# Sir-Teo/MuZero-Go

Hardware: AMD Instinct MI355X
Metric: MCTS simulations/sec (whole node) + self-play moves/sec, 9x9 Go, 200 sims/move (higher is better)
Workload: dtype fp32

## Files before the change

muzero-go_amd/csrc/mzgo_board.hpp:

```cpp
#pragma once
#include "mzgo_common.hpp"

namespace mzgo {

struct BoardMeta {
  int turn;
  int passed;
  int done;
  int moves;
};

template <class G>
struct BoardLds {
  int8_t* stone;
  uint8_t* invd;
  int* label;
  int* libs;
  int* gsize;
  int* killed;
  int* misc;
};

template <class G>
struct BoardWG {
  static constexpr int SIZE = G::THREADS;
  __device__ static int id() { return tid_local(); }
  __device__ static void sync() { __syncthreads(); }
  __device__ static bool any(int v) { return __syncthreads_or(v) != 0; }
  __device__ static bool leader() { return tid_local() == 0; }
};
template <class G>
__device__ __forceinline__ bool nbr(int c, int d, int& n) {
  const int r = c / G::N, col = c - r * G::N;
  switch (d) {
    case 0: if (r == 0) return false; n = c - G::N; return true;
    case 1: if (r == G::N - 1) return false; n = c + G::N; return true;
    case 2: if (col == 0) return false; n = c - 1; return true;
    default: if (col == G::N - 1) return false; n = c + 1; return true;
  }
}

template <class G, class T, class ClassFn>
__device__ __forceinline__ void label_components(int* label, ClassFn cls) {
  for (int c = T::id(); c < G::CELLS; c += T::SIZE) label[c] = cls(c) ? c : -1;
  T::sync();
  for (int it = 0; it < G::CELLS + 2; ++it) {
    int changed = 0;
    for (int c = T::id(); c < G::CELLS; c += T::SIZE) {
      const int k = cls(c);
      if (!k) continue;
      int m = label[c];
#pragma unroll
      for (int d = 0; d < 4; ++d) {
        int n;
        if (nbr<G>(c, d, n) && cls(n) == k) { int ln = label[n]; m = ln < m ? ln : m; }
      }
      int j = label[m];
      m = j < m ? j : m;
      if (m < label[c]) { label[c] = m; changed = 1; }
    }
    if (!T::any(changed)) break;
  }
}

template <class G, class T>
__device__ __forceinline__ void count_liberties(BoardLds<G>& b, bool sizes) {
  for (int c = T::id(); c < G::CELLS; c += T::SIZE) { b.libs[c] = 0; if (sizes) b.gsize[c] = 0; }
  T::sync();
  for (int c = T::id(); c < G::CELLS; c += T::SIZE) {
    if (b.stone[c]) {
      if (sizes) atomicAdd(&b.gsize[b.label[c]], 1);
      continue;
    }
    int seen[4];
    int ns = 0;
#pragma unroll
    for (int d = 0; d < 4; ++d) {
      int n;
      if (nbr<G>(c, d, n) && b.stone[n]) {
        int l = b.label[n];
        bool dup = false;
        for (int i = 0; i < ns; ++i) dup |= seen[i] == l;
        if (!dup) { seen[ns++] = l; atomicAdd(&b.libs[l], 1); }
      }
    }
  }
  T::sync();
}

template <class G, class T>
__device__ __forceinline__ void compute_invalid(BoardLds<G>& b, int mover, int ko) {
  for (int c = T::id(); c < G::CELLS; c += T::SIZE) {
    uint8_t inv;
    if (b.stone[c]) {
      inv = 1;
    } else {
      bool boxed = true, maybe_bad = false, surely_ok = false;
#pragma unroll
      for (int d = 0; d < 4; ++d) {
        int n;
        if (!nbr<G>(c, d, n)) continue;
        const int s = b.stone[n];
        if (!s) { boxed = false; continue; }
        const int lib = b.libs[b.label[n]];
        if (s - 1 == mover) { maybe_bad |= lib > 1; surely_ok |= lib == 1; }
        else                { maybe_bad |= lib == 1; surely_ok |= lib > 1; }
      }
      inv = (boxed && maybe_bad && !surely_ok) ? 1 : 0;
    }
    b.invd[c] = inv;
  }
  T::sync();
  if (ko >= 0 && T::leader()) b.invd[ko] = 1;
  T::sync();
}

enum : int { BOARD_OK = 0, BOARD_ERR_DONE = 1, BOARD_ERR_INVALID = 2, BOARD_ERR_RANGE = 3 };

template <class G, class T = BoardWG<G>>
__device__ __forceinline__ int board_step(BoardLds<G>& b, BoardMeta& m, int action) {
  if (m.done) return BOARD_ERR_DONE;
  if (action < 0 || action > G::CELLS) return BOARD_ERR_RANGE;
  const int player = m.turn;
  int ko = -1;
  if (action == G::CELLS) {
    if (m.passed) m.done = 1;
    m.passed = 1;
    label_components<G, T>(b.label, [&](int c) { return (int)b.stone[c]; });
    count_liberties<G, T>(b, false);
  } else {
    if (b.invd[action]) return BOARD_ERR_INVALID;
    m.passed = 0;
    if (T::leader()) {
      b.stone[action] = (int8_t)(player + 1);
      bool boxed = true;
      for (int d = 0; d < 4; ++d) {
        int n;
        if (nbr<G>(action, d, n)) boxed &= b.stone[n] == 2 - player;
      }
      b.misc[1] = boxed;
    }
    T::sync();
    label_components<G, T>(b.label, [&](int c) { return (int)b.stone[c]; });
    count_liberties<G, T>(b, true);
    if (T::leader()) {
      int nk = 0;
      for (int d = 0; d < 4; ++d) {
        int n;
        if (!nbr<G>(action, d, n) || b.stone[n] != 2 - player) continue;
        const int l = b.label[n];
        bool dup = false;
        for (int i = 0; i < nk; ++i) dup |= b.killed[i] == l;
        if (!dup && b.libs[l] == 0) b.killed[nk++] = l;
      }
      b.misc[0] = nk;
      b.misc[2] = (nk == 1 && b.misc[1] && b.gsize[b.killed[0]] == 1) ? b.killed[0] : -1;
    }
    T::sync();
    const int nk = b.misc[0];
    ko = b.misc[2];
    if (nk > 0) {
      for (int c = T::id(); c < G::CELLS; c += T::SIZE) {
        if (b.stone[c] == 2 - player) {
          const int l = b.label[c];
          bool dead = false;
          for (int i = 0; i < nk; ++i) dead |= b.killed[i] == l;
          if (dead) b.stone[c] = 0;
        }
      }
      T::sync();
      count_liberties<G, T>(b, false);
    }
  }
  compute_invalid<G, T>(b, player, ko);
  m.turn = 1 - m.turn;
  m.moves += 1;
  return BOARD_OK;
}

template <class G, class T = BoardWG<G>>
__device__ __forceinline__ double board_winning(BoardLds<G>& b, double komi) {
  label_components<G, T>(b.label, [&](int c) { return b.stone[c] == 0 ? 1 : 0; });
  for (int c = T::id(); c < G::CELLS; c += T::SIZE) { b.libs[c] = 0; b.gsize[c] = 0; }
  T::sync();
  for (int c = T::id(); c < G::CELLS; c += T::SIZE) {
    if (b.stone[c]) continue;
    int f = 0;
#pragma unroll
    for (int d = 0; d < 4; ++d) {
      int n;
      if (nbr<G>(c, d, n) && b.stone[n]) f |= b.stone[n];
    }
    if (f) atomicOr(&b.libs[b.label[c]], f);
    atomicAdd(&b.gsize[b.label[c]], 1);
  }
  T::sync();
  int black = 0, white = 0;
  for (int c = T::id(); c < G::CELLS; c += T::SIZE) {
    if (b.stone[c] == 1) black++;
    else if (b.stone[c] == 2) white++;
    else if (b.label[c] == c) {
      if (b.libs[c] == 1) black += b.gsize[c];
      else if (b.libs[c] == 2) white += b.gsize[c];
    }
  }
  if (T::leader()) { b.misc[3] = 0; b.misc[4] = 0; }
  T::sync();
  atomicAdd(&b.misc[3], black);
  atomicAdd(&b.misc[4], white);
  T::sync();
  const double diff = (double)b.misc[3] - (double)b.misc[4] - komi;
  T::sync();
  return diff > 0 ? 1.0 : (diff < 0 ? -1.0 : 0.0);
}

}
```

muzero-go_amd/csrc/mzgo_kernels.hpp:

```cpp
#pragma once
#include "mzgo_jobs.hpp"
#include "mzgo_replay.hpp"

namespace mzgo {

template <class G>
constexpr bool rep_needs_scratch() {
  if constexpr (G::WINO) return Wino<G>::NSTRIP > 1;
  else return false;
}

struct NoRepJobs {
  __device__ bool operator()(int) const { return false; }
};

template <class G, class PlaneFn, class Jobs = NoRepJobs>
__device__ __forceinline__ void representation(Smem<G>& sm, const NetParams& np, PlaneFn planes, float* lat,
                                      int lat_stride, float* scr, unsigned long long* ts = nullptr,
                                      Jobs jobs = Jobs{}) {
  float* mid = rep_needs_scratch<G>() ? scr : lat;
  for (int i = tid_local(); i < 6 * G::CELLS; i += G::THREADS) {
    const int c = i / G::CELLS, j = i - c * G::CELLS;
    sm.u.in[c * G::CPAD + j] = planes(c, j);
  }
// ... 1162 lines not shown
  if (tid_local() == 0) {
    E.nodes[g] = nodes;
    atomicAdd(&E.counters[3], (unsigned long long)(factored ? convs : nodes - 1));
    atomicAdd(&E.counters[5], (unsigned long long)(factored ? rows : nodes - 1));
    if (nbcomp) atomicAdd(&E.counters[9], (unsigned long long)nbcomp);
    if (nbcache) atomicAdd(&E.counters[10], (unsigned long long)nbcache);
    if (ncut) atomicAdd(&E.counters[11], (unsigned long long)ncut);
    if (narr_lds) atomicAdd(&E.counters[12], (unsigned long long)narr_lds);
    if (narr_l2) atomicAdd(&E.counters[13], (unsigned long long)narr_l2);
  }
  __syncthreads();
}

template <class G, class PlaneFn>
__device__ __forceinline__ void run_search(Smem<G>& sm, const NetParams& np, const SearchParams& sp,
                                  const EngineArrays& E, int g, PlaneFn planes, const double* noise,
                                  uint64_t key, unsigned long long* ts = nullptr, double* noise_out = nullptr) {
  const TreeView TV = TreeViewOf<G>::make(E, g);
  if (tid_local() == 0) sm.t.ngrab = 0;
  build_mask<G>(sm.t, sp.pass_epsilon, [&](int a) { return planes(3, a); });
  float* pool = pool_of<G>(E, g);
  const size_t node_floats = (size_t)G::C * G::CS;
  if (sp.factored && shared_jobs<G>(sp))
    representation<G>(sm, np, planes, pool + (size_t)(E.S + 1) * node_floats, G::CS, pool, ts ? ts + 3 : nullptr,
                      [&](int k) { rep_shared<G>(sm, np, E, g, sp.net, k); return true; });
  else if (sp.factored)
    representation<G>(sm, np, planes, pool + (size_t)(E.S + 1) * node_floats, G::CS, pool, ts ? ts + 3 : nullptr);
  else
    representation<G>(sm, np, planes, pool, G::CS, pool + node_floats, ts ? ts + 3 : nullptr);
#ifdef MZGO_STAMPS
  if (ts) ts[0] = __builtin_amdgcn_s_memtime();
#endif
  if (noise) {
    if (wave_id() == 0) root_priors<G>(sm.t, TV, sp, noise, key, nullptr, noise_out);
  } else {
    static_assert(G::AP < G::WAVES, "a wave per 64 Gamma draws besides wave 0");
    draw_dirichlet<G>(sm.t, key, sp.dirichlet_alpha, &sm.t.ngrab);
    if (wave_id() == 0) root_priors<G>(sm.t, TV, sp, noise, key, &sm.t.ngrab, noise_out);
  }
  __syncthreads();
#ifdef MZGO_STAMPS
  if (ts) ts[1] = __builtin_amdgcn_s_memtime();
#endif
  if constexpr (G::TREE_CAP > 0) {
    if (sp.num_simulations + 2 <= G::TREE_CAP) {
      sim_loop<G, TreeAcc<G, true>>(sm, np, sp, E, g, TV, key);
      return;
    }
  }
  sim_loop<G, TreeAcc<G, false>>(sm, np, sp, E, g, TV, key);
}

template <class G>
__device__ __forceinline__ void search_outputs(const EngineArrays& E, int g, int* out_visits, double* out_value) {
  const TreeView T = TreeViewOf<G>::make(E, g);
  for (int a = tid_local(); a < G::A; a += G::THREADS) {
    const int c = T.child[a];
    if (out_visits) out_visits[(size_t)g * G::A + a] = c >= 0 ? T.visits[c] : 0;
  }
  if (tid_local() == 0 && out_value) out_value[g] = root_value(T);
}

template <class G>
__device__ __forceinline__ void settle_all_priors(Smem<G>& sm, const NetParams& np, const EngineArrays& E, int g,
                                                  int nodes, int variant) {
  if constexpr (decltype(sm.u.f)::BATCH && G::TREE_CAP > 0) {
    const TreeView TV = TreeViewOf<G>::make(E, g);
    const float* pool = pool_of<G>(E, g);
    const int wave = __builtin_amdgcn_readfirstlane(wave_id());
    const int lane = lane_id_local();
    auto& W = sm.u.f.wv[wave];
    static_assert(sizeof(W.xw) >= sizeof(float) * G::CELLS, "a wave's head rows hold one node's policy sums");
    const int lim = nodes < G::TREE_CAP ? nodes : G::TREE_CAP;
    if (wave == 0 && lane == 0) sm.t.lognode = -1;
    for (int p = wave; p < lim; p += G::WAVES) {
      if (sm.t.is_raw(p)) continue;
      for (int a0 = 0; a0 < G::A; a0 += 64) {
        const int a = a0 + lane;
        const int c = a < G::A ? TV.child[(size_t)p * G::A + a] : -1;
        for (uint64_t m = __ballot(c > 0 && c < lim && sm.t.is_raw(c)); m; m &= m - 1) {
          const int l = __builtin_ctzll(m);
          const int cc = __builtin_amdgcn_readlane(c, l), ca = a0 + l;
          policy_sums_wave<G>(W.xw, pool + (size_t)p * G::C * G::CS, np.etab + (size_t)ca * 9 * G::C, np.head_w);
          wave_lds_sync();
          float x[G::AP], q[G::AP];
          policy_logits<G>(W.xw, sm.t.hsc, x);
          child_prior_regs<G>(sm.t, x, q, variant, W.fb, W.db);
#pragma unroll
          for (int j = 0; j < G::AP; ++j)
            if (lane + 64 * j < G::A) {
              TV.prior[(size_t)cc * G::A + lane + 64 * j] = q[j];
              TV.child[(size_t)cc * G::A + lane + 64 * j] = -1;
            }
          wave_lds_sync();
        }
      }
    }
    __syncthreads();
    for (int i = tid_local(); i < (G::TREE_CAP + 31) / 32; i += G::THREADS) sm.t.rawp[i] = 0u;
  }
  __syncthreads();
}

template <int N, int C>
__global__ void __launch_bounds__((Geo<N, C>::THREADS)) __attribute__((amdgpu_waves_per_eu(Geo<N, C>::WPE, Geo<N, C>::WPE))) k_search(NetParams np_arg, SearchParams sp, EngineArrays E_arg,
                                                      const float* __restrict__ root_obs,
                                                      const double* __restrict__ noise, int game_base,
                                                      int move_index, int* out_visits, double* out_value) {
  typedef Geo<N, C> G;
  __shared__ Smem<G> sm;
  static_assert(sizeof(Smem<G>) <= 160 * 1024, "one workgroup per CU: the whole LDS at most");
  if constexpr (G::WINO) wino_raw_zero<G>(sm.raw);
  const EngineArrays E = launder_arrays(E_arg);
  const NetParams np = launder_params(np_arg);
  const int g = blockIdx.x;
  const float* o = root_obs + (size_t)g * 6 * G::CELLS;
  const uint64_t key = stream_key(sp.seed, (uint32_t)(game_base + g), (uint32_t)move_index);
  run_search<G>(sm, np, sp, E, g, [&](int c, int j) { return o[c * G::CELLS + j]; },
                noise ? noise + (size_t)g * G::A : nullptr, key);
  settle_all_priors<G>(sm, np, E, g, E.nodes[g], sp.variant);
  search_outputs<G>(E, g, out_visits, out_value);
}

template <class G>
__device__ __forceinline__ void board_reset_slot(const EngineArrays& E, int g) {
  for (int c = tid_local(); c < G::CELLS; c += G::THREADS) {
    E.stones[(size_t)g * G::CELLS + c] = 0;
    E.invd[(size_t)g * G::CELLS + c] = 0;
  }
  if (tid_local() < 4) E.meta[g * 4 + tid_local()] = 0;
  if (tid_local() == 0) { E.status[g] = 0; E.game_len[g] = 0; E.final_reward[g] = 0.0; }
}

template <int N, int C>
__global__ void __launch_bounds__((Geo<N, C>::THREADS)) __attribute__((amdgpu_waves_per_eu(Geo<N, C>::WPE, Geo<N, C>::WPE))) k_board_reset(EngineArrays E) {
  board_reset_slot<Geo<N, C>>(E, blockIdx.x);
}

template <int N, int C>
__global__ void __launch_bounds__((Geo<N, C>::THREADS)) __attribute__((amdgpu_waves_per_eu(Geo<N, C>::WPE, Geo<N, C>::WPE))) k_board_step(EngineArrays E, const int* __restrict__ actions,
                                                          int* status, double* winner, double komi) {
  typedef Geo<N, C> G;
  __shared__ Smem<G> sm;
  static_assert(sizeof(Smem<G>) <= 160 * 1024, "one workgroup per CU: the whole LDS at most");
  const int g = blockIdx.x;
  const int a = actions[g];
  if (a < 0) return;
  BoardMeta m;
  board_load<G>(sm.stone, sm.invd, E, g, m);
  BoardLds<G> b = board_lds<G>(sm);
  const int st = board_step<G>(b, m, a);
  __syncthreads();
  if (st == BOARD_OK) board_store<G>(sm.stone, sm.invd, E, g, m);
  double w = 0.0;
  if (st == BOARD_OK && m.done) w = board_winning<G>(b, komi);
  if (tid_local() == 0) {
    if (status) status[g] = st;
    if (winner) winner[g] = w;
  }
}

template <int N, int C>
__global__ void __launch_bounds__((Geo<N, C>::THREADS)) __attribute__((amdgpu_waves_per_eu(Geo<N, C>::WPE, Geo<N, C>::WPE))) k_board_planes(EngineArrays E, double* planes) {
  typedef Geo<N, C> G;
  const int g = blockIdx.x;
  const int* mm = E.meta + g * 4;
  double* p = planes + (size_t)g * 6 * G::CELLS;
  for (int j = tid_local(); j < G::CELLS; j += G::THREADS) {
    const int s = E.stones[(size_t)g * G::CELLS + j];
    p[j] = s == 1; p[G::CELLS + j] = s == 2; p[2 * G::CELLS + j] = mm[0];
    p[3 * G::CELLS + j] = E.invd[(size_t)g * G::CELLS + j];
    p[4 * G::CELLS + j] = mm[1]; p[5 * G::CELLS + j] = mm[2];
  }
}

template <class G, bool CAPS, class KeyId>
__device__ __forceinline__ bool selfplay_one_move(Smem<G>& sm, const NetParams& np_a_arg, const NetParams& np_b_arg,
                                                  const SearchParams& sp, const PlayParams& pp,
                                                  const EngineArrays& E_arg, int g, KeyId key_id, BoardMeta& m) {
#ifdef MZGO_STAMPS
  unsigned long long tm[8] = {0, 0, 0, 0, 0, 0, 0, 0};
  tm[0] = __builtin_amdgcn_s_memtime();
#else
  unsigned long long* tm = nullptr;
#endif
  const int mv = m.moves;
  const EngineArrays E = launder_arrays(E_arg);
  const NetParams np_a = launder_params(np_a_arg), np_b = launder_params(np_b_arg);
  const NetParams np = select_params(pp.arena && (((pp.game_base + g) + mv) & 1), np_b, np_a);
  const size_t rec = (size_t)g * E.max_moves + mv;
  const uint64_t key = move_key(sp, key_id(), mv);
  const int budget = move_budget<CAPS>(sp, key);
  record_observation<G>(E, rec, sm.stone, sm.invd, m, CAPS && budget != sp.num_simulations);
  const BoardMeta m0 = m;
  const double* noise = pp.noise ? pp.noise + ((size_t)g * E.max_moves + mv) * G::A : nullptr;
  double* noise_out = pp.noise_out ? pp.noise_out + ((size_t)g * E.max_moves + mv) * G::A : nullptr;
#ifdef MZGO_STAMPS
  tm[1] = __builtin_amdgcn_s_memtime();
#endif
  SearchParams spm = launder_search(sp);
  spm.net = (pp.arena && (((pp.game_base + g) + mv) & 1)) ? 1 : 0;
  if constexpr (CAPS) spm.num_simulations = budget;
  run_search<G>(sm, np, spm, E, g, [&](int c, int j) { return board_plane<G>(sm.stone, sm.invd, m0, c, j); },
                noise, key, tm ? tm + 2 : nullptr, noise_out);
#ifdef MZGO_STAMPS
  tm[4] = __builtin_amdgcn_s_memtime();
#endif

  const TreeView T = TreeViewOf<G>::make(E, g);
  if (wave_id() == 0) {
    const int a = choose_move_action<G>(sm.t, T, sp, pp, mv, key, E.rec_policy + rec * G::A);
    if (lane_id_local() == 0) {
      sm.bc[0] = a;
      E.rec_action[rec] = a;
      E.rec_value[rec] = root_value(T);
    }
  }
  __syncthreads();
  BoardLds<G> b = board_lds<G>(sm);
  double w;
  const int st = play_action<G>(E, g, b, m, sm.bc[0], pp.komi, w);
#ifdef MZGO_STAMPS
  if (tid_local() == 0 && E.stamps) {
    const unsigned long long t5 = __builtin_amdgcn_s_memtime();
    unsigned long long* sl = E.stamps + (size_t)blockIdx.x * kStampPhases;
    sl[83] += tm[1] - tm[0];
    sl[84] += tm[2] - tm[1];
    sl[85] += tm[3] - tm[2];
    sl[86] += tm[4] - tm[3];
    sl[87] += t5 - tm[4];
    sl[88] += tm[5] - tm[1];
    sl[89] += tm[6] - tm[5];
    sl[90] += tm[2] - tm[6];
  }
#endif
  return finish_move<G>(E, budget, g, rec, st, m, w);
}

template <int N, int C, bool CAPS = false>
__global__ void __launch_bounds__((Geo<N, C>::THREADS)) __attribute__((amdgpu_waves_per_eu(Geo<N, C>::WPE, Geo<N, C>::WPE))) k_selfplay_move(NetParams np_a_arg, NetParams np_b_arg,
                                                             SearchParams sp, PlayParams pp, EngineArrays E_arg) {
  typedef Geo<N, C> G;
  __shared__ Smem<G> sm;
  static_assert(sizeof(Smem<G>) <= 160 * 1024, "one workgroup per CU: the whole LDS at most");
  const int games = gridDim.x - sp.helpers;
  if ((int)blockIdx.x >= games) {
    if constexpr (Smem<G>::GLOBAL_Y && G::WINO) {
      wino_raw_zero<G>(sm.raw);
      int t = (blockIdx.x - games) % games;
      for (;;) {
        helper_loop<G>(sm, np_a_arg, np_b_arg, sp, E_arg, t);
        if (!sp.tail) break;
        t = join_running_game<G>(sm, E_arg, games, t);
        if (t < 0) break;
      }
    }
    return;
  }
  const int g = blockIdx.x;
  const EngineArrays& E = E_arg;
  if (tid_local() == 0) atomicAdd(&E_arg.counters[6], 1ull);
  auto release_helpers = [&]() {
    if ((sp.helpers > 0 || sp.tail) && tid_local() == 0) job_exit(job_of<G>(E_arg, g));
  };
  auto tail_phase = [&]() {
    if constexpr (Smem<G>::GLOBAL_Y && G::WINO) {
      if (sp.tail) {
        __syncthreads();
        for (int t = g; (t = join_running_game<G>(sm, E_arg, games, t)) >= 0;)
          helper_loop<G>(sm, np_a_arg, np_b_arg, sp, E_arg, t);
      }
    }
    if constexpr (TailConvs<G>::value)
      if (sp.tail) {
        __syncthreads();
#ifdef MZGO_STAMPS
        const unsigned long long th = __builtin_amdgcn_s_memtime();
#endif
        tail_help<G>(sm, np_a_arg, np_b_arg, E_arg, g, games);
#ifdef MZGO_STAMPS
        if (tid_local() == 0 && E_arg.stamps) E_arg.stamps[(size_t)blockIdx.x * kStampPhases + 47] +=
            __builtin_amdgcn_s_memtime() - th;
#endif
      }
  };
  if (E.status[g] != 0) { release_helpers(); tail_phase(); return; }
  if ((sp.helpers > 0 || sp.tail) && tid_local() == 0) job_mark_started(job_of<G>(E_arg, g));
  if constexpr (G::WINO) wino_raw_zero<G>(sm.raw);
  BoardMeta m;
  board_load<G>(sm.stone, sm.invd, E, g, m);
  for (int step = 0; step < pp.moves; ++step) {
    if (selfplay_one_move<G, CAPS>(sm, np_a_arg, np_b_arg, sp, pp, E_arg, g,
                             [&]() { return game_key_id(pp.game_base, g, pp.epoch); }, m))
      break;
    __syncthreads();
  }
  release_helpers();
  tail_phase();
}

template <class G>
struct BoardsGeo {
  static constexpr int THREADS = (G::CELLS + 63) / 64 * 64 < 512 ? (G::CELLS + 63) / 64 * 64 : 512;
};
template <class G>
struct BoardsTeam {
  static constexpr int SIZE = BoardsGeo<G>::THREADS;
  __device__ static int id() { return tid_local(); }
  __device__ static void sync() { __syncthreads(); }
  __device__ static bool any(int v) { return __syncthreads_or(v) != 0; }
  __device__ static bool leader() { return tid_local() == 0; }
};
template <class G>
struct BoardsSmem {
  TreeLds<G> t;
  int label[G::CELLS], libs[G::CELLS], gsize[G::CELLS];
  int8_t stone[G::CELLS];
  uint8_t invd[G::CELLS];
  int killed[4];
  int misc[8];
  int bc[8];
};

template <int N, int C, bool CAPS = false>
__global__ void __launch_bounds__((BoardsGeo<Geo<N, C>>::THREADS)) k_selfplay_boards(SearchParams sp, PlayParams pp,
                                                                                    EngineArrays E) {
  typedef Geo<N, C> G;
  typedef BoardsTeam<G> T;
  __shared__ BoardsSmem<G> sm;
  const int g = blockIdx.x;
  const int tid = tid_local();
  if (tid == 0) {
    atomicAdd(&E.counters[6], 1ull);
    E.mpq[2 * g + 1] = 0;
  }
  if (E.status[g] != 0) return;
  BoardMeta m;
  board_load<G, T>(sm.stone, sm.invd, E, g, m);
  BoardLds<G> b = make_board_lds<G>(sm.stone, sm.invd, sm.label, sm.libs, sm.gsize, sm.killed, sm.misc);
  const int mv_first = m.moves;
  int played = 0;
  const TreeView TV = TreeViewOf<G>::make(E, g);
  for (int step = 0; step < pp.moves; ++step) {
    const int mv = m.moves;
    const size_t rec = (size_t)g * E.max_moves + mv;
    const uint64_t key = move_key(sp, pp, g, mv);
    const int budget = move_budget<CAPS>(sp, key);
    record_observation<G, T>(E, rec, sm.stone, sm.invd, m, CAPS && budget != sp.num_simulations);
    ++played;
    build_mask<G, T>(sm.t, sp.pass_epsilon, [&](int a) { return sm.invd[a]; });
    if (wave_id() == 0) {
      const int a = choose_action<G>(sm.t, TV, sp.compat, move_temperature(pp, mv), key, E.rec_policy + rec * G::A);
      if (lane_id_local() == 0) {
        sm.bc[0] = a;
        E.rec_action[rec] = a;
      }
    }
    __syncthreads();
    double w;
    const int st = play_action<G, T>(E, g, b, m, sm.bc[0], pp.komi, w);
    if (finish_move<G, T>(E, budget, g, rec, st, m, w)) break;
    __syncthreads();
  }
  if (tid == 0) {
    E.mpq[2 * g] = mv_first;
    E.mpq[2 * g + 1] = played;
  }
}

template <int N, int C, bool CAPS = false>
__global__ void __launch_bounds__((Geo<N, C>::THREADS)) __attribute__((amdgpu_waves_per_eu(Geo<N, C>::WPE, Geo<N, C>::WPE))) k_search_queue(NetParams np_arg, SearchParams sp, PlayParams pp,
                                                            EngineArrays E_arg, int games) {
  typedef Geo<N, C> G;
  __shared__ Smem<G> sm;
  static_assert(sizeof(Smem<G>) <= 160 * 1024, "one workgroup per CU: the whole LDS at most");
  if constexpr (G::WINO) wino_raw_zero<G>(sm.raw);
  const int leaders = (int)gridDim.x - sp.helpers;
  if ((int)blockIdx.x >= leaders) {
    if constexpr (Smem<G>::GLOBAL_Y && G::WINO)
      helper_loop<G>(sm, np_arg, np_arg, sp, E_arg, ((int)blockIdx.x - leaders) % leaders);
    return;
  }
  const int slot = blockIdx.x;
  const int items = games * pp.moves;
  for (;;) {
    if (tid_local() == 0) sm.bc[0] = (int)atomicAdd((unsigned*)&E_arg.mpq[2 * games], 1u);
    __syncthreads();
    const int k = sm.bc[0];
    __syncthreads();
    if (k >= items) break;
    const int j = k / games, g = k % games;
    const int mv0 = __builtin_amdgcn_readfirstlane(E_arg.mpq[2 * g]);
    const int nmv = __builtin_amdgcn_readfirstlane(E_arg.mpq[2 * g + 1]);
    if (j >= nmv) continue;
    const int mv = mv0 + nmv - 1 - j;
    const EngineArrays E = launder_arrays(E_arg);
    const NetParams np = launder_params(np_arg);
    const size_t rec = (size_t)g * E.max_moves + mv;
    for (int c = tid_local(); c < G::CELLS; c += G::THREADS) {
      sm.stone[c] = E.rec_stones[rec * G::CELLS + c];
      sm.invd[c] = E.rec_invd[rec * G::CELLS + c];
    }
    const BoardMeta m0 = flags_unpack(E.rec_flags[rec], mv);
    __syncthreads();
    const uint64_t key = move_key(sp, pp, g, mv);
    const double* noise = pp.noise ? pp.noise + rec * G::A : nullptr;
    double* noise_out = pp.noise_out ? pp.noise_out + rec * G::A : nullptr;
    SearchParams spm = launder_search(sp);
    spm.net = 0;
    if constexpr (CAPS) spm.num_simulations = move_budget<CAPS>(sp, key);
    run_search<G>(sm, np, spm, E, slot, [&](int c, int jj) { return board_plane<G>(sm.stone, sm.invd, m0, c, jj); },
                  noise, key, nullptr, noise_out);
    if (tid_local() == 0) E.rec_value[rec] = root_value(TreeViewOf<G>::make(E, slot));
    __syncthreads();
  }
  if (sp.helpers > 0 && tid_local() == 0) job_exit(job_of<G>(E_arg, slot));
}

struct ReanalyseArgs {
  const int8_t* stones;
  const uint8_t* invd;
  const uint8_t* flags;
  const int* ids;
  const double* noise;
  int n;
  unsigned* head;
  int* visits;
  double* value;
  double* policy;
};

template <int N, int C, bool INPLACE = false>
__global__ void __launch_bounds__((Geo<N, C>::THREADS)) __attribute__((amdgpu_waves_per_eu(Geo<N, C>::WPE, Geo<N, C>::WPE))) k_reanalyse_queue(NetParams np_arg, SearchParams sp,
                                                               EngineArrays E_arg, typename std::conditional<INPLACE, ReanalyseStoreArgs, ReanalyseArgs>::type ra) {
  typedef Geo<N, C> G;
  __shared__ Smem<G> sm;
  static_assert(sizeof(Smem<G>) <= 160 * 1024, "one workgroup per CU: the whole LDS at most");
  if constexpr (G::WINO) wino_raw_zero<G>(sm.raw);
  const int slot = blockIdx.x;
  if constexpr (INPLACE) {
    for (;;) {
      if (tid_local() == 0) sm.bc[0] = (int)atomicAdd(ra.head, 1u);
      __syncthreads();
      const int i = sm.bc[0];
      __syncthreads();
      if (i >= *launder_global(ra.n)) break;
      const EngineArrays E = launder_arrays(E_arg);
      const NetParams np = launder_params(np_arg);
      const int* it = launder_global(ra.items) + 2 * (size_t)i;
      const int rs = it[0], t = it[1];
      const size_t q = (size_t)rs * (ra.R.M + 1) + t;
      const int8_t* st = launder_global(ra.R.stones) + q * G::CELLS;
      const uint8_t* iv = launder_global(ra.R.invd) + q * G::CELLS;
      for (int c = tid_local(); c < G::CELLS; c += G::THREADS) {
        sm.stone[c] = st[c];
        sm.invd[c] = iv[c];
      }
      const BoardMeta m0 = flags_unpack(launder_global(ra.R.flags)[q], t);
      __syncthreads();
      const uint64_t key = stream_key(sp.seed, (uint32_t)launder_global(ra.R.key_gid)[rs], (uint32_t)t);
      SearchParams spm = launder_search(sp);
      spm.net = 0;
      spm.helpers = 0;
      run_search<G>(sm, np, spm, E, slot, [&](int c, int jj) { return board_plane<G>(sm.stone, sm.invd, m0, c, jj); },
                    nullptr, key);
      const TreeView T = TreeViewOf<G>::make(E, slot);
      const size_t o = (size_t)rs * ra.R.M + t;
      if (tid_local() == 0) {
        launder_global(ra.R.root_value)[o] = root_value(T);
        uint8_t* fl = launder_global(ra.R.flags) + q;
        if (*fl & kFlagFast) *fl = (uint8_t)(*fl & ~kFlagFast);
      }
      if (wave_id() == 0) {
        double vc[G::AP], msum;
        visit_policy<G>(sm.t, T, sp.variant, 1, launder_global(ra.R.policy) + o * G::A, vc, msum);
      }
      __syncthreads();
    }
  } else
  for (;;) {
    if (tid_local() == 0) sm.bc[0] = (int)atomicAdd(ra.head, 1u);
    __syncthreads();
    const int i = sm.bc[0];
    __syncthreads();
    if (i >= ra.n) break;
    const EngineArrays E = launder_arrays(E_arg);
    const NetParams np = launder_params(np_arg);
    const int8_t* st = launder_global(ra.stones) + (size_t)i * G::CELLS;
    const uint8_t* iv = launder_global(ra.invd) + (size_t)i * G::CELLS;
    for (int c = tid_local(); c < G::CELLS; c += G::THREADS) {
      sm.stone[c] = st[c];
      sm.invd[c] = iv[c];
    }
    const int* id = launder_global(ra.ids) + 2 * (size_t)i;
    const BoardMeta m0 = flags_unpack(launder_global(ra.flags)[i], id[1]);
    __syncthreads();
    const uint64_t key = stream_key(sp.seed, (uint32_t)id[0], (uint32_t)id[1]);
    const double* noise = ra.noise ? launder_global(ra.noise) + (size_t)i * G::A : nullptr;
    SearchParams spm = launder_search(sp);
    spm.net = 0;
    spm.helpers = 0;
    run_search<G>(sm, np, spm, E, slot, [&](int c, int jj) { return board_plane<G>(sm.stone, sm.invd, m0, c, jj); },
                  noise, key);
    const TreeView T = TreeViewOf<G>::make(E, slot);
    int* ov = launder_global(ra.visits) + (size_t)i * G::A;
    for (int a = tid_local(); a < G::A; a += G::THREADS) {
      const int c = T.child[a];
      ov[a] = c >= 0 ? T.visits[c] : 0;
    }
    if (tid_local() == 0) launder_global(ra.value)[i] = root_value(T);
    if (ra.policy && wave_id() == 0) {
      double vc[G::AP], msum;
      visit_policy<G>(sm.t, T, sp.variant, 1, launder_global(ra.policy) + (size_t)i * G::A, vc, msum);
    }
    __syncthreads();
  }
}

template <int N, int C, bool CAPS = false>
__global__ void __launch_bounds__((Geo<N, C>::THREADS)) __attribute__((amdgpu_waves_per_eu(Geo<N, C>::WPE, Geo<N, C>::WPE))) k_selfplay_games(NetParams np_arg, SearchParams sp, PlayParams pp,
                                                              EngineArrays E_arg, GamesArgs ga) {
  typedef Geo<N, C> G;
  __shared__ Smem<G> sm;
  static_assert(sizeof(Smem<G>) <= 160 * 1024, "one workgroup per CU: the whole LDS at most");
  if constexpr (G::WINO) wino_raw_zero<G>(sm.raw);
  const int slot = blockIdx.x;
  if (tid_local() == 0) atomicAdd(&E_arg.counters[6], 1ull);
  for (;;) {
    if (tid_local() == 0) sm.bc[0] = (int)atomicAdd(ga.head, 1u);
    __syncthreads();
    const int j = __builtin_amdgcn_readfirstlane(sm.bc[0]);
    __syncthreads();
    if (j >= ga.n) break;
    const uint32_t kid = game_key_id(pp.game_base, j % ga.G, ga.epoch0 + j / ga.G);
    board_reset_slot<G>(E_arg, slot);
    for (int c = tid_local(); c < G::CELLS; c += G::THREADS) {
      sm.stone[c] = 0;
      sm.invd[c] = 0;
    }
    BoardMeta m{0, 0, 0, 0};
    __syncthreads();
    for (int step = 0; step < pp.moves; ++step) {
      if (selfplay_one_move<G, CAPS>(sm, np_arg, np_arg, sp, pp, E_arg, slot, [&]() { return kid; }, m)) break;
      __syncthreads();
    }
    __syncthreads();
    if (tid_local() == 0 && E_arg.status[slot] >= 16) atomicMin(ga.error, j);
    const ReplayEngineView V{N, ga.G, E_arg.max_moves, C, 0, pp.game_base, 0,
                             E_arg.stones, E_arg.invd, E_arg.meta, E_arg.rec_stones, E_arg.rec_invd,
                             E_arg.rec_flags, E_arg.rec_action, E_arg.rec_value, E_arg.rec_policy,
                             E_arg.rec_reward, E_arg.final_reward};
    replay_ingest_game(ga.R, V, slot, (ga.first + j) % ga.R.cap, (int)kid, tid_local(), G::THREADS);
    __syncthreads();
  }
}

}
```

muzero-go_amd/csrc/mzgo_move.hpp:

```cpp
#pragma once
#include "mzgo_board.hpp"
#include "mzgo_search.hpp"

namespace mzgo {

constexpr int kCounters = 14;

struct EngineArrays {
  int S;
  int max_moves;
  float* pool;
  float* prior;
  int* child;
  int* visits;
  double* wsum;
  double* root_prior;
  int* path;
  int* nodes;
  int* nact;
  double* cval;
  int8_t* stones;
  uint8_t* invd;
  int* meta;
  int8_t* rec_stones;
  uint8_t* rec_invd;
  uint8_t* rec_flags;
  int* rec_action;
  double* rec_value;
  double* rec_policy;
  double* rec_reward;
  int* game_len;
  double* final_reward;
  int* status;
  unsigned char* jobs;
  int* mpq;
  unsigned long long* counters;
  unsigned long long* stamps;
};

struct PlayParams {
  double temperature;
  int temperature_moves;
  double komi;
  int game_base;
  int epoch;
  const double* noise;
  double* noise_out;
  int arena;
  int moves;
};

template <class G>
__device__ __forceinline__ BoardLds<G> make_board_lds(int8_t* stone, uint8_t* invd, int* label, int* libs,
                                                      int* gsize, int* killed, int* misc) {
  return BoardLds<G>{stone, invd, label, libs, gsize, killed, misc};
}

template <class G, class T = BoardWG<G>>
__device__ __forceinline__ void board_load(int8_t* stone, uint8_t* invd, const EngineArrays& E, int g,
                                           BoardMeta& m) {
  for (int c = T::id(); c < G::CELLS; c += T::SIZE) {
    stone[c] = E.stones[(size_t)g * G::CELLS + c];
    invd[c] = E.invd[(size_t)g * G::CELLS + c];
  }
  const int* mm = E.meta + g * 4;
  m.turn = mm[0]; m.passed = mm[1]; m.done = mm[2]; m.moves = mm[3];
  T::sync();
}

template <class G, class T = BoardWG<G>>
__device__ __forceinline__ void board_store(const int8_t* stone, const uint8_t* invd, const EngineArrays& E, int g,
                                            const BoardMeta& m) {
  for (int c = T::id(); c < G::CELLS; c += T::SIZE) {
    E.stones[(size_t)g * G::CELLS + c] = stone[c];
    E.invd[(size_t)g * G::CELLS + c] = invd[c];
  }
  if (T::leader()) {
    int* mm = E.meta + g * 4;
    mm[0] = m.turn; mm[1] = m.passed; mm[2] = m.done; mm[3] = m.moves;
  }
}

template <class G>
__device__ __forceinline__ float board_plane(const int8_t* stone, const uint8_t* invd, const BoardMeta& m, int c,
                                             int j) {
  switch (c) {
    case 0: return stone[j] == 1 ? 1.f : 0.f;
    case 1: return stone[j] == 2 ? 1.f : 0.f;
    case 2: return (float)m.turn;
    case 3: return (float)invd[j];
    case 4: return (float)m.passed;
    default: return (float)m.done;
  }
}

__device__ __forceinline__ uint8_t flags_pack(const BoardMeta& m) {
  return (uint8_t)(m.turn | (m.passed << 1) | (m.done << 2));
}
__device__ __forceinline__ BoardMeta flags_unpack(int fl, int mv) {
  return BoardMeta{fl & 1, (fl >> 1) & 1, (fl >> 2) & 1, mv};
}

constexpr int kFlagFast = 8;

template <class G, class T = BoardWG<G>>
__device__ __forceinline__ void record_observation(const EngineArrays& E, size_t rec, const int8_t* stone,
                                                   const uint8_t* invd, const BoardMeta& m, bool fast = false) {
  for (int c = T::id(); c < G::CELLS; c += T::SIZE) {
    E.rec_stones[rec * G::CELLS + c] = stone[c];
    E.rec_invd[rec * G::CELLS + c] = invd[c];
  }
  if (T::leader()) E.rec_flags[rec] = (uint8_t)(flags_pack(m) | (fast ? kFlagFast : 0));
}

__host__ __device__ __forceinline__ uint32_t game_key_id(int game_base, int g, int epoch) {
  return (uint32_t)(game_base + g) ^ ((uint32_t)epoch << 24);
}
__device__ __forceinline__ uint64_t move_key(const SearchParams& sp, uint32_t kid, int mv) {
  return stream_key(sp.seed, kid, (uint32_t)mv);
}
__device__ __forceinline__ uint64_t move_key(const SearchParams& sp, const PlayParams& pp, int g, int mv) {
  return move_key(sp, game_key_id(pp.game_base, g, pp.epoch), mv);
}

template <bool CAPS>
__device__ __forceinline__ int move_budget(const SearchParams& sp, uint64_t key) {
  if constexpr (!CAPS) return sp.num_simulations;
  else return __builtin_amdgcn_readfirstlane(
      playout_budget(key, sp.num_simulations, sp.fast_simulations, sp.full_search_prob));
}

template <class G, class T = BoardWG<G>, class InvdFn>
__device__ __forceinline__ void build_mask(TreeLds<G>& t, double pass_epsilon, InvdFn invd) {
  int any = 0;
  for (int a = T::id(); a < G::A; a += T::SIZE) {
    uint8_t v = a < G::CELLS ? (invd(a) == 0 ? 1 : 0) : 1;
    t.valid[a] = v;
    any |= (a < G::CELLS) && v;
  }
  any = T::any(any);
  if (T::leader()) t.pass_prior = any ? pass_epsilon : 1.0;
  T::sync();
}

template <class G>
__device__ __forceinline__ int pick_valid(const TreeLds<G>& t, uint64_t h) {
  const int lane = lane_id_local();
  uint64_t vb[G::AP];
  int nvalid = 0;
#pragma unroll
  for (int j = 0; j < G::AP; ++j) {
    const int a = lane + 64 * j;
    vb[j] = __ballot(a < G::A && mask_of<G>(t, a) > 0);
    nvalid += __popcll(vb[j]);
  }
  uint32_t k = randbelow(h, (uint32_t)nvalid);
  int action = -1;
#pragma unroll
  for (int j = 0; j < G::AP; ++j) {
    const uint32_t c = __popcll(vb[j]);
    if (action < 0 && k < c) {
      uint64_t mm = vb[j];
      for (uint32_t i = 0; i < k; ++i) mm &= mm - 1;
      action = 64 * j + __ffsll((long long)mm) - 1;
    } else if (action < 0) {
      k -= c;
    }
  }
  return action;
}

template <class G>
__device__ __forceinline__ int argmax_action(const double (&v)[G::AP]) {
  const int lane = lane_id_local();
  double bv = -1.0;
  int ba = 0x7fffffff, payload = 0;
#pragma unroll
  for (int j = 0; j < G::AP; ++j) {
    const int a = lane + 64 * j;
    if (a < G::A && (v[j] > bv || (v[j] == bv && a < ba))) { bv = v[j]; ba = a; }
  }
  wave_argmax(bv, ba, payload);
  return ba;
}

template <class G>
__device__ __forceinline__ double visit_policy(TreeLds<G>& t, const TreeView& T, int variant, int compat,
                                               double* pol, double (&vc)[G::AP], double& msum) {
  const int lane = lane_id_local();
  if (variant == 1) {
    double tot = 0.0;
#pragma unroll
    for (int j = 0; j < G::AP; ++j) {
      const int a = lane + 64 * j;
      vc[j] = 0.0;
      if (a < G::A && mask_of<G>(t, a) > 0) { const int c = T.child[a]; vc[j] = c >= 0 ? (double)T.visits[c] : 0.0; }
      tot += vc[j];
    }
    tot = wave_sum(tot);
#pragma unroll
    for (int j = 0; j < G::AP; ++j) {
      const int a = lane + 64 * j;
      if (a < G::A) pol[a] = tot > 0 ? vc[j] / tot : 0.0;
    }
    msum = 0.0;
    return tot;
  }
  for (int a = lane; a < G::A; a += 64) {
    double v = 0.0;
    if (compat == 1) { const int c = T.child[a]; v = c >= 0 ? (double)T.visits[c] : 0.0; }
    t.dbuf[a] = v * mask_of<G>(t, a);
  }
  wave_lds_sync();
  const double vsum = np_pairwise_sum<double, G::A>(t.dbuf);
#pragma unroll
  for (int j = 0; j < G::AP; ++j) { const int a = lane + 64 * j; vc[j] = a < G::A ? t.dbuf[a] : 0.0; }
  wave_lds_sync();
  for (int a = lane; a < G::A; a += 64) t.dbuf[a] = mask_of<G>(t, a);
  wave_lds_sync();
  msum = np_pairwise_sum<double, G::A>(t.dbuf);
#pragma unroll
  for (int j = 0; j < G::AP; ++j) {
    const int a = lane + 64 * j;
    if (a < G::A) pol[a] = vsum > 0 ? vc[j] / vsum : mask_of<G>(t, a) / msum;
  }
  return vsum;
}

template <class G>
__device__ __forceinline__ int choose_action_main(TreeLds<G>& t, const TreeView& T, uint64_t key, double* pol) {
  const int lane = lane_id_local();
  double vc[G::AP], msum;
  const double tot = visit_policy<G>(t, T, 1, 1, pol, vc, msum);
  if (tot > 0) return argmax_action<G>(vc);
  const int action = pick_valid<G>(t, draw(key, TAG_ACTION, 0));
#pragma unroll
  for (int j = 0; j < G::AP; ++j) {
    const int a = lane + 64 * j;
    if (a < G::A) pol[a] = a == action ? 1.0 : 0.0;
  }
  return action;
}

template <class G>
__device__ __forceinline__ int choose_action(TreeLds<G>& t, const TreeView& T, int compat, double temperature,
                                    uint64_t key, double* pol) {
  const int lane = lane_id_local();
  double vcm[G::AP], msum;
  const double vsum = visit_policy<G>(t, T, 0, compat, pol, vcm, msum);
  const uint64_t h = draw(key, TAG_ACTION, 0);
  if (temperature == 0.0) return vsum > 0 ? argmax_action<G>(vcm) : pick_valid<G>(t, h);
  const double e = 1.0 / temperature;
#pragma unroll
  for (int j = 0; j < G::AP; ++j) {
    const int a = lane + 64 * j;
    if (a < G::A) t.dbuf[a] = (e == 1.0 ? vcm[j] : pow(vcm[j], e)) * mask_of<G>(t, a);
  }
  wave_lds_sync();
  const double ts = np_pairwise_sum<double, G::A>(t.dbuf);
  wave_lds_sync();
  for (int a = lane; a < G::A; a += 64) t.dbuf[a] = ts > 0 ? t.dbuf[a] / ts : mask_of<G>(t, a) / msum;
  wave_lds_sync();
  if (lane == 0) {
    double cdf = 0.0;
    for (int a = 0; a < G::A; ++a) cdf += t.dbuf[a];
    const double total = cdf;
    const double u = u01(h);
    double run = 0.0;
    int idx = 0;
    for (int a = 0; a < G::A; ++a) {
      run += t.dbuf[a];
      if (run / total <= u) idx = a + 1;
    }
    t.bcast = idx;
  }
  wave_lds_sync();
  return t.bcast;
}

__device__ __forceinline__ double move_temperature(const PlayParams& pp, int mv) {
  return mv < pp.temperature_moves ? pp.temperature : 0.0;
}
template <class G>
__device__ __forceinline__ int choose_move_action(TreeLds<G>& t, const TreeView& T, const SearchParams& sp,
                                                  const PlayParams& pp, int mv, uint64_t key, double* pol) {
  return sp.variant == 1 ? choose_action_main<G>(t, T, key, pol)
                         : choose_action<G>(t, T, sp.compat, move_temperature(pp, mv), key, pol);
}

__device__ __forceinline__ double root_value(const TreeView& T) {
  const int n = T.visits[0];
  return n > 0 ? T.wsum[0] / (double)n : 0.0;
}

template <class G, class T = BoardWG<G>>
__device__ __forceinline__ int play_action(const EngineArrays& E, int g, BoardLds<G>& b, BoardMeta& m, int action,
                                           double komi, double& w) {
  const int st = board_step<G, T>(b, m, action);
  T::sync();
  w = (st == BOARD_OK && m.done) ? board_winning<G, T>(b, komi) : 0.0;
  board_store<G, T>(b.stone, b.invd, E, g, m);
  return st;
}

template <class G, class T = BoardWG<G>>
__device__ __forceinline__ bool finish_move(const EngineArrays& E, int sims, int g, size_t rec, int st,
                                            const BoardMeta& m, double w) {
  const bool ended = m.done || m.moves >= E.max_moves;
  if (T::leader()) {
    E.rec_reward[rec] = w;
    atomicAdd(&E.counters[0], (unsigned long long)sims);
    atomicAdd(&E.counters[1], 1ull);
    if (st != BOARD_OK) {
      E.status[g] = 16 + st;
    } else if (ended) {
      E.status[g] = 1;
      E.game_len[g] = m.moves;
      E.final_reward[g] = m.done ? w : 0.0;
      atomicAdd(&E.counters[2], 1ull);
    }
  }
  return st != BOARD_OK || ended;
}

}
```

Baseline: 143.1 million.

## Incrementally update board groups, lighten barriers, and batch move counters in the board loop

The multi-move board loop now keeps group labels across moves: it merges neighbouring friendly labels directly instead of rerunning iterative connected-component labelling on every stone placement, and the board is stored to global memory only once at the end. The team sync and any-reduction use wave-level syncs or raw s_barrier with per-wave flags instead of __syncthreads/__syncthreads_or. Global atomics for the sim, move and game counters are accumulated locally and flushed once per game. The temperature sampling in choose_action is rewritten as a wave-parallel prefix scan with a ballot instead of a serial lane-0 loop. These changes cut per-move synchronisation, global traffic and labelling passes, at the cost of more complex invariants: labels must stay consistent after captures and passes, and the rewritten CDF summation order may change floating-point rounding.

Result: faster. 144.7 million (median of 6 runs) (+1.2%).

```diff
diff --git a/muzero-go_amd/csrc/mzgo_board.hpp b/muzero-go_amd/csrc/mzgo_board.hpp
--- a/muzero-go_amd/csrc/mzgo_board.hpp
+++ b/muzero-go_amd/csrc/mzgo_board.hpp
@@ -26,7 +26,7 @@
   static constexpr int SIZE = G::THREADS;
   __device__ static int id() { return tid_local(); }
   __device__ static void sync() { __syncthreads(); }
-  __device__ static bool any(int v) { return __syncthreads_or(v) != 0; }
+  __device__ static bool any(int v, int = 0) { return __syncthreads_or(v) != 0; }
   __device__ static bool leader() { return tid_local() == 0; }
 };
 template <class G>
@@ -59,7 +59,7 @@
       m = j < m ? j : m;
       if (m < label[c]) { label[c] = m; changed = 1; }
     }
-    if (!T::any(changed)) break;
+    if (!T::any(changed, it)) break;
   }
 }
 
@@ -117,7 +117,13 @@
 
 enum : int { BOARD_OK = 0, BOARD_ERR_DONE = 1, BOARD_ERR_INVALID = 2, BOARD_ERR_RANGE = 3 };
 
-template <class G, class T = BoardWG<G>>
+template <class G, class T>
+__device__ __forceinline__ void board_groups(BoardLds<G>& b) {
+  label_components<G, T>(b.label, [&](int c) { return (int)b.stone[c]; });
+  count_liberties<G, T>(b, false);
+}
+
+template <class G, class T = BoardWG<G>, bool KEEP = false>
 __device__ __forceinline__ int board_step(BoardLds<G>& b, BoardMeta& m, int action) {
   if (m.done) return BOARD_ERR_DONE;
   if (action < 0 || action > G::CELLS) return BOARD_ERR_RANGE;
@@ -126,11 +132,21 @@
   if (action == G::CELLS) {
     if (m.passed) m.done = 1;
     m.passed = 1;
-    label_components<G, T>(b.label, [&](int c) { return (int)b.stone[c]; });
-    count_liberties<G, T>(b, false);
+    if constexpr (!KEEP) board_groups<G, T>(b);
   } else {
     if (b.invd[action]) return BOARD_ERR_INVALID;
     m.passed = 0;
+    int join[4] = {-2, -2, -2, -2}, lmin = action;
+    if constexpr (KEEP) {
+#pragma unroll
+      for (int d = 0; d < 4; ++d) {
+        int n;
+        if (nbr<G>(action, d, n) && b.stone[n] == player + 1) {
+          join[d] = b.label[n];
+          lmin = join[d] < lmin ? join[d] : lmin;
+        }
+      }
+    }
     if (T::leader()) {
       b.stone[action] = (int8_t)(player + 1);
       bool boxed = true;
@@ -141,7 +157,16 @@
       b.misc[1] = boxed;
     }
     T::sync();
-    label_components<G, T>(b.label, [&](int c) { return (int)b.stone[c]; });
+    if constexpr (KEEP) {
+      for (int c = T::id(); c < G::CELLS; c += T::SIZE) {
+        if (c == action) { b.label[c] = lmin; continue; }
+        if (b.stone[c] != player + 1) continue;
+        const int l = b.label[c];
+        if (l == join[0] || l == join[1] || l == join[2] || l == join[3]) b.label[c] = lmin;
+      }
+    } else {
+      label_components<G, T>(b.label, [&](int c) { return (int)b.stone[c]; });
+    }
     count_liberties<G, T>(b, true);
     if (T::leader()) {
       int nk = 0;
@@ -165,7 +190,7 @@
           const int l = b.label[c];
           bool dead = false;
           for (int i = 0; i < nk; ++i) dead |= b.killed[i] == l;
-          if (dead) b.stone[c] = 0;
+          if (dead) { b.stone[c] = 0; if constexpr (KEEP) b.label[c] = -1; }
         }
       }
       T::sync();
diff --git a/muzero-go_amd/csrc/mzgo_kernels.hpp b/muzero-go_amd/csrc/mzgo_kernels.hpp
--- a/muzero-go_amd/csrc/mzgo_kernels.hpp
+++ b/muzero-go_amd/csrc/mzgo_kernels.hpp
@@ -1488,13 +1488,37 @@
 template <class G>
 struct BoardsGeo {
   static constexpr int THREADS = (G::CELLS + 63) / 64 * 64 < 512 ? (G::CELLS + 63) / 64 * 64 : 512;
+  static constexpr int WAVES = THREADS / 64;
 };
 template <class G>
 struct BoardsTeam {
   static constexpr int SIZE = BoardsGeo<G>::THREADS;
+  static constexpr int WAVES = BoardsGeo<G>::WAVES;
   __device__ static int id() { return tid_local(); }
-  __device__ static void sync() { __syncthreads(); }
-  __device__ static bool any(int v) { return __syncthreads_or(v) != 0; }
+  __device__ static void sync() {
+    if constexpr (WAVES == 1) {
+      wave_lds_sync();
+    } else {
+      __builtin_amdgcn_fence(__ATOMIC_RELEASE, "workgroup", "local");
+      __builtin_amdgcn_s_barrier();
+      __builtin_amdgcn_fence(__ATOMIC_ACQUIRE, "workgroup", "local");
+    }
+  }
+  __device__ static bool any(int v, int phase = 0) {
+    const bool mine = __ballot(v != 0) != 0;
+    if constexpr (WAVES == 1) {
+      wave_lds_sync();
+      return mine;
+    } else {
+      __shared__ int flag[2][WAVES];
+      if (lane_id_local() == 0) flag[phase & 1][wave_id()] = mine;
+      sync();
+      int r = 0;
+#pragma unroll
+      for (int w = 0; w < WAVES; ++w) r |= flag[phase & 1][w];
+      return r != 0;
+    }
+  }
   __device__ static bool leader() { return tid_local() == 0; }
 };
 template <class G>
@@ -1524,8 +1548,20 @@
   BoardMeta m;
   board_load<G, T>(sm.stone, sm.invd, E, g, m);
   BoardLds<G> b = make_board_lds<G>(sm.stone, sm.invd, sm.label, sm.libs, sm.gsize, sm.killed, sm.misc);
+  board_groups<G, T>(b);
+#ifdef MZGO_STAMPS
+  unsigned long long lapc[6] = {}, lapt = __builtin_amdgcn_s_memtime();
+  auto lap = [&](int k) {
+    const unsigned long long now = __builtin_amdgcn_s_memtime();
+    lapc[k] += now - lapt;
+    lapt = now;
+  };
+#else
+  auto lap = [](int) {};
+#endif
   const int mv_first = m.moves;
-  int played = 0;
+  int played = 0, finished = 0;
+  unsigned long long sims = 0;
   const TreeView TV = TreeViewOf<G>::make(E, g);
   for (int step = 0; step < pp.moves; ++step) {
     const int mv = m.moves;
@@ -1533,8 +1569,11 @@
     const uint64_t key = move_key(sp, pp, g, mv);
     const int budget = move_budget<CAPS>(sp, key);
     record_observation<G, T>(E, rec, sm.stone, sm.invd, m, CAPS && budget != sp.num_simulations);
+    lap(0);
     ++played;
+    sims += (unsigned long long)budget;
     build_mask<G, T>(sm.t, sp.pass_epsilon, [&](int a) { return sm.invd[a]; });
+    lap(1);
     if (wave_id() == 0) {
       const int a = choose_action<G>(sm.t, TV, sp.compat, move_temperature(pp, mv), key, E.rec_policy + rec * G::A);
       if (lane_id_local() == 0) {
@@ -1542,13 +1581,26 @@
         E.rec_action[rec] = a;
       }
     }
-    __syncthreads();
+    T::sync();
+    lap(move_temperature(pp, mv) != 0.0 ? 2 : 3);
     double w;
-    const int st = play_action<G, T>(E, g, b, m, sm.bc[0], pp.komi, w);
-    if (finish_move<G, T>(E, budget, g, rec, st, m, w)) break;
-    __syncthreads();
-  }
+    const int st = play_action<G, T, true>(E, g, b, m, sm.bc[0], pp.komi, w);
+    lap(4);
+    finished += game_finished(E, st, m);
+    if (finish_move<G, T, false>(E, budget, g, rec, st, m, w)) break;
+    T::sync();
+    lap(5);
+  }
+  board_store<G, T>(sm.stone, sm.invd, E, g, m);
   if (tid == 0) {
+    count_moves(E, sims, played, finished);
+#ifdef MZGO_STAMPS
+    if (E.stamps) {
+      unsigned long long* row = E.stamps + (size_t)g * kStampPhases;
+      row[83] += lapc[0]; row[84] += lapc[1]; row[85] += lapc[2]; row[86] += lapc[3];
+      row[87] += lapc[4]; row[47] += lapc[5]; row[45] += (unsigned long long)played;
+    }
+#endif
     E.mpq[2 * g] = mv_first;
     E.mpq[2 * g + 1] = played;
   }
diff --git a/muzero-go_amd/csrc/mzgo_move.hpp b/muzero-go_amd/csrc/mzgo_move.hpp
--- a/muzero-go_amd/csrc/mzgo_move.hpp
+++ b/muzero-go_amd/csrc/mzgo_move.hpp
@@ -259,23 +259,32 @@
   wave_lds_sync();
   const double ts = np_pairwise_sum<double, G::A>(t.dbuf);
   wave_lds_sync();
-  for (int a = lane; a < G::A; a += 64) t.dbuf[a] = ts > 0 ? t.dbuf[a] / ts : mask_of<G>(t, a) / msum;
-  wave_lds_sync();
-  if (lane == 0) {
-    double cdf = 0.0;
-    for (int a = 0; a < G::A; ++a) cdf += t.dbuf[a];
-    const double total = cdf;
-    const double u = u01(h);
-    double run = 0.0;
-    int idx = 0;
-    for (int a = 0; a < G::A; ++a) {
-      run += t.dbuf[a];
-      if (run / total <= u) idx = a + 1;
-    }
-    t.bcast = idx;
-  }
-  wave_lds_sync();
-  return t.bcast;
+  double p[G::AP], pre[G::AP];
+#pragma unroll
+  for (int j = 0; j < G::AP; ++j) {
+    const int a = lane + 64 * j;
+    p[j] = a < G::A ? (ts > 0 ? t.dbuf[a] / ts : mask_of<G>(t, a) / msum) : 0.0;
+    pre[j] = 0.0;
+  }
+  double run = 0.0;
+#pragma unroll
+  for (int j = 0; j < G::AP; ++j) {
+#pragma unroll
+    for (int l = 0; l < 64; ++l) {
+      if (64 * j + l < G::A) {
+        run += dpp::lane(p[j], l);
+        if (lane == l) pre[j] = run;
+      }
+    }
+  }
+  const double total = run, u = u01(h);
+  int idx = 0;
+#pragma unroll
+  for (int j = 0; j < G::AP; ++j) {
+    const uint64_t ok = __ballot(lane + 64 * j < G::A && pre[j] / total <= u);
+    if (ok) idx = 64 * j + 64 - __clzll((long long)ok);
+  }
+  return idx;
 }
 
 __device__ __forceinline__ double move_temperature(const PlayParams& pp, int mv) {
@@ -293,34 +302,46 @@
   return n > 0 ? T.wsum[0] / (double)n : 0.0;
 }
 
-template <class G, class T = BoardWG<G>>
+template <class G, class T = BoardWG<G>, bool HELD = false>
 __device__ __forceinline__ int play_action(const EngineArrays& E, int g, BoardLds<G>& b, BoardMeta& m, int action,
                                            double komi, double& w) {
-  const int st = board_step<G, T>(b, m, action);
+  const int st = board_step<G, T, HELD>(b, m, action);
   T::sync();
   w = (st == BOARD_OK && m.done) ? board_winning<G, T>(b, komi) : 0.0;
-  board_store<G, T>(b.stone, b.invd, E, g, m);
+  if constexpr (!HELD) board_store<G, T>(b.stone, b.invd, E, g, m);
   return st;
 }
 
-template <class G, class T = BoardWG<G>>
+template <class G, class T = BoardWG<G>, bool COUNT = true>
 __device__ __forceinline__ bool finish_move(const EngineArrays& E, int sims, int g, size_t rec, int st,
                                             const BoardMeta& m, double w) {
   const bool ended = m.done || m.moves >= E.max_moves;
   if (T::leader()) {
     E.rec_reward[rec] = w;
-    atomicAdd(&E.counters[0], (unsigned long long)sims);
-    atomicAdd(&E.counters[1], 1ull);
+    if constexpr (COUNT) {
+      atomicAdd(&E.counters[0], (unsigned long long)sims);
+      atomicAdd(&E.counters[1], 1ull);
+    }
     if (st != BOARD_OK) {
       E.status[g] = 16 + st;
     } else if (ended) {
       E.status[g] = 1;
       E.game_len[g] = m.moves;
       E.final_reward[g] = m.done ? w : 0.0;
-      atomicAdd(&E.counters[2], 1ull);
+      if constexpr (COUNT) atomicAdd(&E.counters[2], 1ull);
     }
   }
   return st != BOARD_OK || ended;
 }
-
-}
+__device__ __forceinline__ bool game_finished(const EngineArrays& E, int st, const BoardMeta& m) {
+  return st == BOARD_OK && (m.done || m.moves >= E.max_moves);
+}
+__device__ __forceinline__ void count_moves(const EngineArrays& E, unsigned long long sims, int moves, int finished) {
+  if (moves) {
+    atomicAdd(&E.counters[0], sims);
+    atomicAdd(&E.counters[1], (unsigned long long)moves);
+  }
+  if (finished) atomicAdd(&E.counters[2], (unsigned long long)finished);
+}
+
+}
```
